# Clemapfel/egg_fluid_simulation

Hardware: AMD Instinct MI355X
Metric: pair_solves_per_sec (higher is better)
Workload: dtype f64

## Files before the change

### egg_fluid_simulation_amd/csrc/eggsim_device.h

```cpp
#pragma once
#include <stdint.h>

#define EGG_MAX_PASSES 64
#define EGG_WAVE 64

struct EggStatus {
    int32_t fail_claim;
    int32_t fail_overflow;
    int32_t fail_stall;
    int32_t fail_range;
    int32_t min_slack;
    int32_t was_cut;
    int32_t fail_levels;
    int32_t max_level;
    int32_t fail_levlds;
    int32_t reserved0;
    unsigned long long visits[EGG_MAX_PASSES];
    unsigned long long max_list;
    unsigned long long rounds;
};

struct EggStepArgs {
    const double *x_in, *y_in, *vx_in, *vy_in;
    double *x_out, *y_out, *vx_out, *vy_out;
// ... 95 lines not shown
    uint32_t *pk_ckey;
    int32_t pk_stride;
    uint32_t *lists;
    uint16_t *lvl;
    uint32_t *rank;
    uint32_t *sorted;
    uint32_t *chunks;
    int32_t *grp_nchunks;
    uint32_t *lev_start;
    int32_t *grp_nlev;
    int32_t *tile_total;
    int32_t *tile_visits;
    int32_t *tile_need;
    int32_t *tile_slack;
    int32_t *tile_fast;
    int32_t lcap, scap, lev_cap, sort_cap, chunk_cap;
    int32_t nmax, amax, ccap, use_grid, stage_cap;
    double sub_delta, damping, follow_compliance, collision_compliance, overlap_factor, cell_size, eps;
    int32_t n_substeps, n_collision_steps;
    int32_t pass_seq, substep, stale;
    int32_t tune;
    uint32_t *simd_claims;
    int32_t lev_lds_cap;
    EggStatus *status, *status_next;
};
#define EGG_PK_MAX_PASSES 64
#define EGG_PK_WINDOW 128

static inline size_t egg_pk_lists_lds_bytes(int nmax, int amax, int ccap, int use_grid, int stage_cap, int gens) {
    size_t n = (size_t)nmax, a = (size_t)amax, c = (size_t)ccap, b = 0, G = (size_t)gens;
    b += egg_align16(G * n * 4);
    b += egg_align16(G * c * 4);
    b += egg_align16(use_grid ? 0 : G * c * 4);
    b += egg_align16((n + 1) * 4);
    b += egg_align16(n * 4);
    b += egg_align16(a * 4 * 4);
    b += egg_align16((a + 1) * 4);
    b += egg_align16(16 * 4);
    b += egg_align16(G * n * 2);
    b += egg_align16(n * 2);
    {
        const size_t stage = egg_align16(((size_t)stage_cap + 1) * (n + 1) * 2), tmp = egg_align16(n * 4) + egg_align16(n * 2);
        b += stage > tmp ? stage : tmp;
    }
    return b;
}
// ... 751 lines not shown
```

### egg_fluid_simulation_amd/csrc/eggsim_host.h

```cpp
#pragma once
#include <hip/hip_runtime.h>

#include <algorithm>
#include <chrono>
#include <cmath>
#include <cstdarg>
#include <cstdio>
#include <cstdlib>
#include <cstring>
#include <functional>
#include <limits>
#include <memory>
#include <numeric>
#include <string>
#include <vector>

#include "../../include/eggsim.h"
#include "eggsim_device.h"

extern "C" __global__ void egg_step_kernel(EggStepArgs A);
extern "C" __global__ void egg_step_kernel_gl(EggStepArgs A);
extern "C" __global__ void egg_step_kernel_occ(EggStepArgs A);
extern "C" __global__ void egg_step_kernel_wide(EggStepArgs A);
extern "C" __global__ void egg_env_bounds_kernel(const double *, const double *, const double *, const double *, const double *, int,
// ... 207 lines not shown
    int nmax = 0, amax = 0, ccap = 0, use_grid = 0, lcap = 0;
    int global_lists = 0;
    int global_state = 0;
    int threads = 0;
    int wide = 0;
    int pair_cache = 0;
    size_t scratch_stride = 0;
    size_t lds = 0, scratch_offset = 0;
    int packed = -1;
};

struct PackedClass {
    int cls = 0;
    int n_tiles = 0, n_groups = 0;
    int p_begin = 0, p_end = 0;
    int tile_base = 0;
    int group_base = 0;
    size_t meta_tile_geo = 0, meta_grp_geo = 0;
    int max_group_particles = 0;
    int fused_pass = 0;
    size_t lds_pass = 0;
    int lev_lds_cap = 0;
    int lev_lds_now = 0;
    size_t lds_levels_now = 0, lds_pass_now = 0;
    int max_tiles_in_group = 0;
    int levels_ooo = 0;
    int levels_threads = 64;
    int lcap = 0, scap = 0;
    int stage_cap = 0;
    int sort_cap = 0;
    size_t sort_base = 0;
    int chunk_cap = 0;
    size_t chunk_base = 0;
    size_t lds_sort = 0;
    size_t entry_base = 0;
    size_t lds_lists = 0, lds_lists_stale = 0, lds_levels = 0, lds_exec = 0;
    int threads_lists = 64, threads_lists_stale = 64;
};

struct RelaxedBufs {
    DevBuf<double2> pos, pos_next, prev, spos, swr;
    DevBuf<int32_t> pslot, tmp, sidx, p_atom;
    DevBuf<unsigned long long> hkey, status;
    DevBuf<uint32_t> hcount, hstart;
    DevBuf<double> targets;
    DevBuf<unsigned char> scan_tmp;
    size_t scan_bytes = 0;
    uint32_t table = 0;
    uint64_t atoms_gen = ~0ull;
// ... 60 lines not shown
    int single_tile = 0;
    int uncut_streak = 0;
    double list_factor = 6.0;
    size_t list_min = 0;
    bool has_env = false;
    double env_min_mass = 0, env_max_mass = 0, env_min_radius = 0, env_max_radius = 0;
    double tiled_cell_size = 0;
    double step_follow_compliance = 57.6, step_damping = 0.9;
    int step_substeps = 2;
    bool pk_allowed = true;
    std::vector<PackedClass> pk;
    std::vector<int32_t> pk_meta_host;
    DevBuf<int32_t> pk_meta, pk_src, pk_atom, pk_tile, pk_nchunks;
    DevBuf<double> pk_pos, pk_prev, pk_wr;
    DevBuf<uint32_t> pk_ckey, pk_lists, pk_rank, pk_sorted, pk_levstart, pk_chunks;
    size_t pk_chunk_words = 0;
    DevBuf<uint16_t> pk_lvl, pk_aslot;
    size_t pk_meta_claims = 0;
    int pk_n = 0, pk_tiles = 0, pk_groups = 0;
    size_t pk_entries = 0;
    size_t pk_sort_words = 0;
    int pk_lev_cap = 255;
    int pk_seen_levels = 0;
    unsigned long long pk_seen_list = 0;
    size_t pk_lev_lds_min = 0;
    bool pk_plan_dirty = true;
    struct PkStamp { hipEvent_t a, b; int kind, launches; };
    std::vector<PkStamp> pk_stamps;
    size_t pk_stamps_used = 0;
    EggStatus *h_status = nullptr;
    RelaxedBufs rx;
    hipStream_t stream = nullptr;
    hipEvent_t ev0 = nullptr, ev1 = nullptr;
};

constexpr size_t kStatInts = 160;
static_assert(sizeof(EggStatus) <= kStatInts * 4, "status block too small");
inline EggStatus *d_stat(System &s, int parity) { return (EggStatus *)(s.d_out.p + parity * kStatInts); }
inline int32_t *d_aabb(System &s) { return s.d_out.p + 2 * kStatInts; }
inline int32_t *d_disp(System &s) { return s.d_out.p + 2 * kStatInts + 4 * s.atoms.size(); }

}
namespace egghost {
struct WireStep;
struct DrawSource;
struct InstanceState;
struct SensorState;
struct ProbeState;
// ... 221 lines not shown
int for_each_requested_atom(egg_handle *h, const char *name, int mask, int64_t n_ids, const int64_t *ids, Fn fn) {
    const std::vector<int32_t> atom_of = atom_of_batch(h);
    for (int64_t i = 0; i < n_ids; ++i) {
        const int32_t a = atom_of[(size_t)(find_batch(h, ids[i]) - h->batches.data())];
        for (int w = 0; w < 2; ++w) {
            if (!(mask >> w & 1) || a < 0) continue;
            const Atom &at = h->sys[w].atoms[(size_t)a];
            if (at.count < 1) continue;
            if (at.offset < 0 || (int64_t)at.offset + at.count > h->sys[w].n)
                return fail(h, EGG_ERR_INTERNAL, "%s: atom %d of type %d holds %d particles from %d", name, (int)a, w, (int)at.count, (int)at.offset);
            const int rc = fn(at, w, (int32_t)(2 * i + w));
            if (rc != EGG_OK) return rc;
        }
    }
    return EGG_OK;
}
typedef egg_sensor egg_region;
int check_region(egg_handle *h, const char *what, int32_t k, egg_region &o);
double cell_size_of(const egg_config &c);
int fetch_end_aabb(egg_handle *h, System &s);

extern double g_retile_ms[8];
int retile(egg_handle *h, int which);

struct Env {
    double sub_delta, damping, follow_c, collision_c, budget, cell;
    double cohesion_c;
};
Env make_env(const egg_config &c, double sub_delta, int64_t n);
enum { kWhole = 0, kPrepare = 1, kBegin = 2, kEnd = 3 };
int do_step(egg_handle *h, double delta, int S, int C, int phase = kWhole);
int follow_config(egg_handle *h, int w, bool launch);

constexpr int64_t kRelaxedMaxParticles = (int64_t)1 << 29;
#define EGG_RX_TOO_MANY_TEXT "relaxed order: more than 2^29 particles of one type"
constexpr char kRelaxedBadCellText[] = "relaxed order: a position is NaN or its spatial-hash cell lies outside +-2^30";
struct RelaxedLayout {
    size_t P = 0, nq = 0;
    bool halo = false;
    bool cohesion = false;
    bool colliders = false;
    bool forces = false;
    size_t V = 0;
    bool surfaces = false;
    bool walls = false;
    bool motion = false;
// ... 86 lines not shown
```

### egg_fluid_simulation_amd/csrc/eggsim_host_step.hip

```cpp
#include "eggsim_host.h"

namespace egghost {


Env make_env(const egg_config &c, double sub_delta, int64_t n) {
    Env e;
    e.sub_delta = sub_delta;
    auto compliance = [&](double strength) {
        double alpha = 1 - clampd(strength, 0, 1);
        return alpha / (sub_delta * sub_delta);
    };
    e.damping = 1 - clampd(c.damping, 0, 1);
    e.follow_c = compliance(c.follow_strength);
    e.collision_c = compliance(c.collision_strength);
    e.cohesion_c = compliance(c.cohesion_strength);
    double nn = (double)n;
    e.budget = c.max_collision_fraction * (nn * nn);
    e.cell = cell_size_of(c);
    return e;
}

int launch_prologue(egg_handle *h, int which, hipStream_t stream) {
    System &s = h->sys[which];
    s.parity ^= 1;
// ... 152 lines not shown
    A.scap = pc.scap;
    A.lev_cap = s.pk_lev_cap;
    A.sort_cap = pc.sort_cap;
    A.chunk_cap = pc.chunk_cap;
    A.stage_cap = pc.stage_cap;
    A.nmax = lc.nmax;
    A.amax = lc.amax;
    A.ccap = lc.ccap;
    A.use_grid = lc.use_grid;
    if (!lc.use_grid) h->stats.cell_hash[which]++;
    A.sub_delta = env.sub_delta;
    A.damping = env.damping;
    A.follow_compliance = env.follow_c;
    A.collision_compliance = env.collision_c;
    A.overlap_factor = s.cfg.collision_overlap_factor;
    A.cell_size = env.cell;
    A.eps = s.cfg.eps;
    A.n_substeps = S;
    A.n_collision_steps = C;
    A.status = d_stat(s, s.parity);
    A.status_next = d_stat(s, s.parity ^ 1);
    A.tune = h->opt_tune;
    A.lev_lds_cap = pc.lev_lds_now;
    A.simd_claims = h->simd_claims.p;
}

int launch_packed(egg_handle *h, int which, const Env &env, int S, int C) {
    System &s = h->sys[which];
    const hipStream_t st = s.stream;
    if (s.pk_plan_dirty) {
        HIP_TRY(h, hipMemcpyAsync(s.pk_meta.p, s.pk_meta_host.data(), s.pk_meta_host.size() * sizeof(int32_t),
                                  hipMemcpyHostToDevice, st));
    }
    for (PackedClass &pc : s.pk) {
        if (!pc.levels_ooo) continue;
        int now = pc.lev_lds_cap;
        if (s.pk_seen_list) now = (int)std::min<size_t>((size_t)now, std::max<size_t>((size_t)(s.pk_seen_list + s.pk_seen_list / 4 + 256), s.pk_lev_lds_min));
        now = std::min(pc.lev_lds_cap, (now + 7) & ~7);
        pc.lev_lds_now = now;
        pc.lds_levels_now = egg_pk_levels_ooo_lds_bytes(s.pk_lev_cap, pc.max_group_particles, pc.max_tiles_in_group, now);
        pc.lds_pass_now = std::max(pc.lds_levels_now, pc.lds_exec + 64 * 16 + (size_t)EGG_PK_RING_BYTES);
    }
    std::vector<EggPackedArgs> args(s.pk.size());
    for (size_t k = 0; k < s.pk.size(); ++k) fill_packed_args(h, which, s.pk[k], env, S, C, args[k]);
    const bool stamp = h->opt_timing >= 2;
    s.pk_stamps_used = 0;
    auto stamp_begin = [&](int kind) -> System::PkStamp * {
        if (!stamp) return nullptr;
        if (s.pk_stamps_used == s.pk_stamps.size()) {
            System::PkStamp ps{nullptr, nullptr, 0, 0};
            if (hipEventCreate(&ps.a) != hipSuccess || hipEventCreate(&ps.b) != hipSuccess) return nullptr;
            s.pk_stamps.push_back(ps);
        }
        System::PkStamp *ps = &s.pk_stamps[s.pk_stamps_used++];
        ps->kind = kind;
        ps->launches = (int)s.pk.size();
        (void)hipEventRecord(ps->a, st);
        return ps;
    };
    auto launch_some = [&](int take, int kind, auto kernel_of, auto grid_of, auto block_of, auto lds_of) {
        System::PkStamp *ps = nullptr;
        for (size_t k = 0; k < s.pk.size(); ++k) {
            const PackedClass &pc = s.pk[k];
// ... 327 lines not shown
                return fail(h, EGG_ERR_INTERNAL, "pair scheduler stalled (type %d, %s)", w,
                            st.fail_stall == 2 ? "time limit reached"
                            : st.fail_stall == 3 ? "workgroup narrower than the wide kernel needs"
                            : st.fail_stall == 4 ? "a wait between the waves of the packed pipeline did not end"
                                                 : "a particle's pair sequence did not finish");
            if (st.fail_overflow) {
                s.list_min = std::max<size_t>(s.list_min, (size_t)(st.max_list * 5 / 4 + 64));
                s.list_factor *= 1.5;
                if (s.list_min > (size_t)kMaxGlobalListEntries)
                    return fail(h, EGG_ERR_UNSUPPORTED, "a tile visits %llu pairs in one pass; limit is %d",
                                (unsigned long long)st.max_list, kMaxGlobalListEntries);
                s.tiling_dirty = true;
                redo = true;
                continue;
            }
            if (st.fail_levlds) {
                s.pk_lev_lds_min = std::max<size_t>(s.pk_lev_lds_min, (size_t)(st.max_list * 5 / 4 + 256));
                s.pk_seen_list = std::max(s.pk_seen_list, st.max_list);
                s.tiling_dirty = true;
                redo = true;
                continue;
            }
            if (st.fail_levels) {
                s.pk_lev_cap = std::max(2 * s.pk_lev_cap + 1, st.max_level + 64);
                if (s.pk_lev_cap > 65535)
                    return fail(h, EGG_ERR_UNSUPPORTED, "a pair-dependency chain of %d levels in one pass; limit is 65535", st.max_level);
                s.tiling_dirty = true;
                redo = true;
                continue;
            }
            if (st.fail_claim || st.fail_range) {
                std::vector<int32_t> failed(s.atoms.size());
                if (!failed.empty()) {
                    HIP_TRY(h, hipMemcpyAsync(failed.data(), s.d_atom_fail.p, failed.size() * sizeof(int32_t),
                                              hipMemcpyDeviceToHost, s.stream));
                    HIP_TRY(h, hipStreamSynchronize(s.stream));
                }
                s.extra_margin.resize(h->batches.size(), 0);
                bool any = false;
                for (size_t k = 0; k < failed.size(); ++k)
                    if (failed[k]) {
                        int &e = s.extra_margin[(size_t)s.atoms[k].batch];
                        e = std::min(4096, std::max(2, 2 * e));
                        any = true;
                    }
                if (!any) s.margin = std::min(s.margin + std::max(2, s.margin / 2), 4096);
// ... 15 lines not shown
                        break;
                    }
            }
        }
        if (redo) {
            h->stats.redo_steps++;
            continue;
        }
        for (int w = 0; w < 2; ++w) {
            System &s = h->sys[w];
            if (s.n == 0 || s.classes.empty()) continue;
            const EggStatus &st = *s.h_status;
            s.cur ^= 1;
            const int np = std::min(S * C, EGG_MAX_PASSES);
            int64_t most = 0;
            for (int p = 0; p < np; ++p) {
                h->stats.pair_solves += (int64_t)st.visits[p];
                most = std::max(most, (int64_t)st.visits[p]);
            }
            h->stats.max_pass_visits[w] = most;
            h->stats.max_levels[w] = s.pk.empty() ? 0 : st.max_level;
            if (!s.pk.empty()) {
                s.pk_seen_list = st.max_list;
                s.pk_seen_levels = st.max_level;
                s.pk_lev_lds_min = 0;
            }
#ifdef EGG_PROFILE
            if (getenv("EGGSIM_DEBUG") && !s.pk.empty())
                fprintf(stderr, "eggsim: type %d step %lld, last pass, egg_pk_levels_ooo cycles: group 0 init %llu rank %llu walk %llu finish %llu sort %llu total %llu | slowest group: walk %llu total %llu | turns %llu levels %d\n",
                        w, (long long)h->stats.steps, st.visits[55], st.visits[56], st.visits[57], st.visits[58], st.visits[59], st.visits[60], st.visits[61], st.visits[62], st.rounds, st.max_level);
            if (getenv("EGGSIM_DEBUG") && !s.pk.empty()) {
                fprintf(stderr, "   group 0 wave 0: %llu turns; cycles waiting for the batch's entries %llu, in the batch set-up %llu, in the turns %llu\n", st.visits[38], st.visits[36], st.visits[39], st.visits[37]);
                fprintf(stderr, "   executor of group 0: %llu cycles for %llu chunks = %.1f per chunk; slowest group %.1f per chunk\n", st.visits[30], st.visits[31],
                        (double)st.visits[30] / (double)std::max<unsigned long long>(st.visits[31], 1), (double)st.visits[32] / 16.0);
                fprintf(stderr, "   executor of group 0: %llu ticks of the 100 MHz clock, i.e. the cycle counter ran at %.0f MHz\n", st.visits[28], st.visits[28] ? 100.0 * (double)st.visits[30] / (double)st.visits[28] : 0.0);
                fprintf(stderr, "   executor of group 0 looked at the helper's progress %llu times and spent %llu cycles there\n", st.visits[26], st.visits[27]);
                fprintf(stderr, "   executor waves on SIMD 0 / 1 / 2 (all passes of the step): %llu %llu %llu; without a SIMD of their own: %llu\n", st.visits[33], st.visits[34], st.visits[35], st.visits[29]);
                fprintf(stderr, "   groups by total cycles (25k buckets):");
                for (int k = 0; k < 15; ++k) fprintf(stderr, " %llu", st.visits[40 + k]);
                fprintf(stderr, "\n");
            }
#endif
            h->stats.budget[w] = env[w].budget;
            h->stats.follow_solves += s.n * S;
            s.aabb_on_device = true;
            if (s.out_copied) {
                const size_t na = s.atoms.size();
                s.aabb.resize(na);
// ... 5 lines not shown
            } else {
                s.aabb_valid = false;
                s.disp_valid = false;
            }
            if (st.min_slack < std::max(1, s.margin - 1) || s.swept) s.tiling_dirty = true;
            if (s.padded && ++s.since_tiling >= 8) s.tiling_dirty = true;
            if (s.margin > h->opt_margin) {
                s.margin -= 1;
                s.tiling_dirty = true;
            }
            for (int &e : s.extra_margin)
                if (e > 0) {
                    e -= 1;
                    s.tiling_dirty = true;
                }
            if (s.single_tile && !h->opt_force_single) {
                s.uncut_streak = st.was_cut ? 0 : s.uncut_streak + 1;
                if (s.uncut_streak >= 8) {
                    s.single_tile = 0;
                    s.tiling_dirty = true;
                }
            }
            h->stats.single_tile[w] = s.single_tile;
            s.eager_boxes = s.tiling_dirty || s.claims_stale || s.targets_moving;
        }
        h->stats.last_step_kernel_ms = ms;
        for (int w = 0; w < 2; ++w) {
            System &s = h->sys[w];
            h->stats.packed[w] = (int64_t)s.pk.size();
            h->stats.pk_variants[w] = 0;
            for (const PackedClass &pc : s.pk)
                h->stats.pk_variants[w] |= (pc.levels_ooo ? EGG_PK_VARIANT_LEVELS_OOO : EGG_PK_VARIANT_LEVELS_INORDER) |
                                           (pc.n_groups <= 4 * std::max(1, h->prop.multiProcessorCount) ? EGG_PK_VARIANT_EXEC_CHAIN : EGG_PK_VARIANT_EXEC) |
                                           (pc.levels_ooo ? 0 : pc.lds_sort ? EGG_PK_VARIANT_SORT_LDS : EGG_PK_VARIANT_SORT_DIRECT) |
                                           (pc.fused_pass ? EGG_PK_VARIANT_PASS_FUSED : 0);
            for (size_t k = 0; h->opt_timing >= 2 && k < s.pk_stamps_used; ++k) {
                const System::PkStamp &ps = s.pk_stamps[k];
                float t = 0;
                if (ps.kind >= 0 && hipEventElapsedTime(&t, ps.a, ps.b) == hipSuccess) {
                    h->stats.pk_kernel_ms[w][ps.kind] += (double)t;
                    h->stats.pk_kernel_launches[w][ps.kind] += ps.launches;
                }
            }
            s.pk_stamps_used = 0;
        }
        if (h->opt_timing) {
// ... 10 lines not shown
```

### egg_fluid_simulation_amd/csrc/eggsim_host_tiling.hip

```cpp
#include "eggsim_host.h"

namespace egghost {




double g_retile_ms[8];
struct RetileLap {
    std::chrono::steady_clock::time_point t = std::chrono::steady_clock::now();
    void operator()(int k) {
        const auto n = std::chrono::steady_clock::now();
        g_retile_ms[k] += std::chrono::duration<double, std::milli>(n - t).count();
        t = n;
    }
};

static size_t pk_admitted_blocks(egg_handle *h, const void *kernel, int threads, size_t lds) {
    for (const egg_handle::PkResidency &r : h->pk_residency)
        if (r.kernel == kernel && r.threads == threads && r.lds == lds) return r.blocks > 0 ? (size_t)r.blocks : SIZE_MAX;
    int blocks = 0;
    const hipError_t e = hipOccupancyMaxActiveBlocksPerMultiprocessor(&blocks, kernel, threads, lds);
    if (e != hipSuccess || blocks <= 0) {
        (void)hipGetLastError();
        blocks = 0;
        if (!h->pk_residency_warned)
            fprintf(stderr, "eggsim: no residency answer for a list kernel at %d threads, %zu B LDS (%s): thread counts are chosen by the LDS / wave model alone\n",
                    threads, lds, hipGetErrorString(e));
        h->pk_residency_warned = true;
    }
    h->pk_residency.push_back({kernel, threads, lds, blocks});
    return blocks > 0 ? (size_t)blocks : SIZE_MAX;
}

static size_t pk_lists_admitted(egg_handle *h, int gens, int threads, size_t lds) {
    const bool fold = !(h->opt_tune & 128);
    if (gens == 2)
        return pk_admitted_blocks(h, fold ? (const void *)egg_pk_lists_stale_mid_kernel : (const void *)egg_pk_lists_stale_kernel, threads, lds);
    const size_t plain = pk_admitted_blocks(h, (const void *)egg_pk_lists_fresh_kernel, threads, lds);
    return fold ? std::min(plain, pk_admitted_blocks(h, (const void *)egg_pk_lists_first_kernel, threads, lds)) : plain;
}

int retile(egg_handle *h, int which) {
    System &s = h->sys[which];
    RetileLap lap;
    int rc = upload_atoms(h, which);
    if (rc != EGG_OK) return rc;
    const size_t na = s.atoms.size();
    const double cell = cell_size_of(s.cfg);
    s.extra_margin.resize(h->batches.size(), 0);
    s.tile_atom_begin.assign(1, 0);
    s.tile_atoms.clear();
    s.classes.clear();
    h->stats.n_tiles[which] = 0;
    h->stats.max_tile_particles[which] = 0;
    if (na == 0) {
        s.tiling_dirty = false;
        s.tiled_cell_size = cell;
        return EGG_OK;
    }
    if (!s.aabb_valid && s.aabb_on_device && s.tiled_cell_size == cell) {
        rc = fetch_end_aabb(h, s);
        if (rc != EGG_OK) return rc;
// ... 408 lines not shown
            }
            const int64_t gp_max = std::max<int64_t>(h->opt_group_particles > 0 ? h->opt_group_particles : gp_auto,
                                                     tiles[(size_t)lc.first_tile].particles);
            int max_tiles_in_group = 0;
            for (int t = 0; t < lc.n_tiles;) {
                int64_t in_group = 0;
                int t_end = t;
                while (t_end < lc.n_tiles && t_end - t < 64) {
                    const int64_t np = tiles[(size_t)lc.first_tile + t_end].particles;
                    if (t_end > t && (in_group + np > gp_max || in_group + np > 32767)) break;
                    in_group += np;
                    ++t_end;
                }
                const int32_t rec[4] = {t, t_end, tile_first_particle[(size_t)t], (int32_t)in_group};
                s.pk_meta_host.insert(s.pk_meta_host.end(), rec, rec + 4);
                pc.n_groups++;
                pc.max_group_particles = std::max<int>(pc.max_group_particles, (int)in_group);
                max_tiles_in_group = std::max(max_tiles_in_group, t_end - t);
                t = t_end;
            }
            const int simds = 4 * std::max(1, h->prop.multiProcessorCount);
            const bool dense_tiles = tiles[(size_t)lc.first_tile].particles > 256;
            pc.levels_ooo = h->lds_lane_ordered && h->opt_level_walk != 1 && (h->opt_level_walk == 2 || (pc.n_groups <= simds && dense_tiles));
            if (pc.levels_ooo) {
                const size_t guess = s.pk_seen_list ? (size_t)(s.pk_seen_list * 3 / 2 + 512) : (size_t)24 * lc.nmax;
                pc.lev_lds_cap = (int)std::min<size_t>((size_t)pc.scap, std::max<size_t>(guess, s.pk_lev_lds_min));
                pc.lev_lds_cap = (pc.lev_lds_cap + 7) & ~7;
                if (pc.n_groups > std::max(1, h->prop.multiProcessorCount)) {
                    const size_t budget = (kLdsMax - 4096) / 2;
                    const size_t fixed = egg_pk_levels_ooo_lds_bytes(s.pk_lev_cap, pc.max_group_particles, max_tiles_in_group, 0);
                    if (budget > fixed) {
                        const size_t fit = ((budget - fixed) / ((size_t)max_tiles_in_group * 2)) & ~(size_t)7;
                        const size_t need = std::max<size_t>((size_t)(s.pk_seen_list + s.pk_seen_list / 16 + 64), s.pk_lev_lds_min);
                        if (fit >= need && (size_t)pc.lev_lds_cap > fit) pc.lev_lds_cap = (int)fit;
                    }
                }
                pc.levels_threads = 64 * std::min(16, std::max(4, max_tiles_in_group <= 4 ? 2 * max_tiles_in_group : max_tiles_in_group));
                pc.lds_levels = egg_pk_levels_ooo_lds_bytes(s.pk_lev_cap, pc.max_group_particles, max_tiles_in_group, pc.lev_lds_cap);
                if (pc.lds_levels > h->lds_limit) pc.levels_ooo = 0;
            }
            pc.fused_pass = pc.levels_ooo && pc.levels_threads <= 512 && max_tiles_in_group <= 4 && pc.n_groups <= simds && !(h->opt_tune & 64);
            if (!pc.levels_ooo) {
                pc.levels_threads = std::min(256, (max_tiles_in_group * 16 + 63) / 64 * 64);
                pc.lds_levels = egg_pk_levels_mr_lds_bytes(s.pk_lev_cap, pc.max_group_particles, pc.levels_threads);
            }
            const size_t sort_words = (size_t)max_tiles_in_group * (size_t)pc.scap + 64;
            pc.chunk_cap = (int)std::min<size_t>(sort_words / 64 + (size_t)s.pk_lev_cap + 8, (size_t)1 << 28);
            pc.lds_exec = (size_t)pc.max_group_particles * 16;
            pc.lds_sort = egg_align16((size_t)(s.pk_lev_cap + 2) * 4) + sort_words * 4;
            if (pc.lds_sort > 64 * 1024) pc.lds_sort = 0;
            if (pc.lds_exec + 64 * 16 > h->lds_limit || pc.lds_levels > h->lds_limit || sort_words >= ((size_t)1 << 26)) {
                s.pk_meta_host.resize(meta_mark);
                continue;
            }
            if (pc.fused_pass) {
                pc.lds_pass = std::max(pc.lds_levels, pc.lds_exec + 64 * 16 + (size_t)EGG_PK_RING_BYTES);
                if (pc.lds_pass > h->lds_limit) pc.fused_pass = 0;
            }
            pc.sort_cap = (int)sort_words;
            pc.max_tiles_in_group = max_tiles_in_group;
            pc.lev_lds_now = pc.lev_lds_cap;
            pc.lds_levels_now = pc.lds_levels;
            pc.lds_pass_now = pc.lds_pass;
            if (getenv("EGGSIM_DEBUG"))
                fprintf(stderr, "eggsim: type %d packed class: %d tiles of <= %d particles in %d groups, grid cells %d (%s), lists: %d threads, %d staged partners, %zu B LDS; levels: %s, %d threads, %zu B LDS (level array %d entries); pass fused %d, %zu B LDS\n",
                        which, lc.n_tiles, lc.nmax, pc.n_groups, lc.ccap, lc.use_grid ? "dense grid" : "hash", pc.threads_lists, pc.stage_cap, pc.lds_lists,
                        pc.levels_ooo ? "out of order" : "in order", pc.levels_threads, pc.lds_levels, pc.lev_lds_cap, pc.fused_pass, pc.lds_pass);
            pc.chunk_base = s.pk_chunk_words;
            s.pk_chunk_words += (size_t)pc.n_groups * (size_t)pc.chunk_cap;
            lc.packed = (int)s.pk.size();
            s.pk_n = pn;
            s.pk_tiles += lc.n_tiles;
            s.pk_groups += pc.n_groups;
            s.pk_entries += (size_t)lc.n_tiles * (size_t)pc.scap;
            s.pk_sort_words += (size_t)pc.n_groups * (size_t)pc.sort_cap;
            s.pk.push_back(pc);
        }
        if (!s.pk.empty()) {
            s.pk_meta_claims = (s.pk_meta_host.size() + 3) & ~(size_t)3;
            s.pk_meta_host.resize(s.pk_meta_claims);
            for (int32_t a : s.tile_atoms) {
                const Box &c = claim[(size_t)a];
                const int32_t rec[4] = {c.lo_x, c.lo_y, c.hi_x, c.hi_y};
                s.pk_meta_host.insert(s.pk_meta_host.end(), rec, rec + 4);
            }
            lap(5);
            const size_t np = (size_t)s.pk_n, nt = (size_t)s.pk_tiles, ng = (size_t)s.pk_groups;
            HIP_TRY(h, s.pk_meta.reserve(s.pk_meta_host.size() + 4, false, s.stream));
            HIP_TRY(h, s.pk_src.reserve(np, false, s.stream));
            HIP_TRY(h, s.pk_atom.reserve(np, false, s.stream));
            HIP_TRY(h, s.pk_aslot.reserve(np + 8, false, s.stream));
            HIP_TRY(h, s.pk_pos.reserve(2 * np, false, s.stream));
            HIP_TRY(h, s.pk_prev.reserve(2 * np, false, s.stream));
            HIP_TRY(h, s.pk_wr.reserve(2 * np, false, s.stream));
            HIP_TRY(h, s.pk_ckey.reserve(2 * np, false, s.stream));
            HIP_TRY(h, s.pk_lists.reserve(s.pk_entries + 64, false, s.stream));
            HIP_TRY(h, s.pk_lvl.reserve(s.pk_entries + 64, false, s.stream));
            bool any_ooo = false;
            for (const PackedClass &pc : s.pk) any_ooo |= pc.levels_ooo != 0;
            if (any_ooo) HIP_TRY(h, s.pk_rank.reserve(s.pk_entries + 64, false, s.stream));
            HIP_TRY(h, s.pk_sorted.reserve(s.pk_sort_words + 64, false, s.stream));
            HIP_TRY(h, s.pk_chunks.reserve(s.pk_chunk_words + 64, false, s.stream));
            HIP_TRY(h, s.pk_nchunks.reserve(2 * ng + 8, false, s.stream));
            HIP_TRY(h, s.pk_levstart.reserve(ng * ((size_t)s.pk_lev_cap + 2) + 64, false, s.stream));
            HIP_TRY(h, s.pk_tile.reserve(nt * (3 + 2 * EGG_PK_MAX_PASSES) + 4, false, s.stream));
        }
        s.pk_plan_dirty = true;
    }

    HIP_TRY(h, s.d_scratch.reserve(scratch_bytes + 16, false, s.stream));
    lap(6);
    s.h_claim = claim;
    s.meta_dirty = true;
    s.tiling_dirty = false;
    h->stats.retiles++;
    h->stats.n_tiles[which] = (int64_t)tiles.size();
    h->stats.max_tile_particles[which] = tiles.empty() ? 0 : tiles.front().particles;
    lap(7);
    return EGG_OK;
}

}
```

### egg_fluid_simulation_amd/csrc/eggsim_packed.hip

```cpp
#include <hip/hip_runtime.h>
#include "eggsim_device.h"

#include "eggsim_tile.h"

namespace {


__device__ inline uint32_t pk_cell_meta(const Tile &t, int gh, int buf, uint32_t key) {
    if (t.use_grid) return t.cell(buf)[(int)(key >> 16) * gh + (int)(key & 0xFFFFu)];
    return cell_meta(t, buf, key);
}

template <class F>
__device__ inline int pk_visit_fresh(const Tile &t, int gh, int cur, int i, F emit) {
    const uint32_t ki = t.ckey(cur)[i];
    const uint16_t *items = t.hitems(cur);
    int count = 0;
    if (t.use_grid) {
        const uint32_t *cells = t.cell(cur);
        const int h1 = (int)(ki >> 16) * gh + (int)(ki & 0xFFFFu);
#pragma unroll
        for (int p = 0; p < 3; ++p) {
            const int h0 = h1 + (p - 1) * gh - 1;
            const uint32_t m0 = cells[h0], m2 = cells[h0 + 2];
// ... 397 lines not shown
            } else {
                pk_visit_fresh(t, gh, cur, i, emit);
            }
        }
    }
#pragma unroll
    for (int d = 32; d >= 1; d >>= 1) guarded += __shfl_xor(guarded, d, 64);
    if ((tid & 63) == 0) wtot[tid >> 6] = guarded;
    __syncthreads();
    if (tid == 0) {
        uint32_t gsum = 0;
        for (int w = 0; w < (nthreads + 63) / 64; ++w) gsum += wtot[w];
        A.tile_visits[(size_t)min(A.pass_seq, EGG_PK_MAX_PASSES - 1) * A.n_tiles + tile] =
            (fits && !any_bad) ? total - (int)gsum : 0;
    }
}
#define EGG_PK_LISTS_KERNEL extern "C" __global__ void __launch_bounds__(1024) __attribute__((amdgpu_num_sgpr(72)))
EGG_PK_LISTS_KERNEL egg_pk_lists_fresh_kernel(EggPackedArgs A) { egg_pk_lists_body<false, false>(A, blockIdx.x); }
EGG_PK_LISTS_KERNEL egg_pk_lists_stale_kernel(EggPackedArgs A) { egg_pk_lists_body<true, false>(A, blockIdx.x); }
EGG_PK_LISTS_KERNEL egg_pk_lists_first_kernel(EggPackedArgs A) { egg_pk_lists_body<false, true>(A, blockIdx.x); }
EGG_PK_LISTS_KERNEL egg_pk_lists_stale_mid_kernel(EggPackedArgs A) { egg_pk_lists_body<true, true>(A, blockIdx.x); }


__device__ __forceinline__ bool pk_levels_finish(const EggPackedArgs &A, int g, const uint32_t *hist, int maxlev, bool over, int lane, uint32_t *cursor = nullptr) {
    const int lev_cap = A.lev_cap;
    if (over && lane == 0) atomicExch(&A.status->fail_levels, 1);
    if (lane == 0 && maxlev > __hip_atomic_load(&A.status->max_level, __ATOMIC_RELAXED, __HIP_MEMORY_SCOPE_AGENT))
        atomicMax(&A.status->max_level, maxlev);
    const int nlev = min(maxlev, lev_cap);
    uint32_t *lstart = A.lev_start + (size_t)g * (lev_cap + 2);
    uint32_t *chunks = A.chunks + (size_t)g * A.chunk_cap;
    uint32_t carry = 0, ccarry = 0;
    for (int b0 = 1; b0 <= nlev; b0 += 64) {
        const int L = b0 + lane;
        const uint32_t v = (L <= nlev) ? hist[L] : 0u;
        const uint32_t nch = (v + 63u) >> 6;
        const uint32_t incl = (uint32_t)wave_incl_scan((int)v, lane), cincl = (uint32_t)wave_incl_scan((int)nch, lane);
        const uint32_t start = carry + incl - v, cb = ccarry + cincl - nch;
        if (L <= nlev) {
            lstart[L] = start;
            if (cursor) cursor[L] = start;
            for (uint32_t c = 0; c < nch; ++c)
                if (cb + c < (uint32_t)A.chunk_cap) chunks[cb + c] = (start + 64u * c) | ((min(64u, v - 64u * c) - 1u) << 26);
        }
        carry += (uint32_t)__builtin_amdgcn_readlane((int)incl, 63);
        ccarry += (uint32_t)__builtin_amdgcn_readlane((int)cincl, 63);
    }
    const bool usable = !over && ccarry <= (uint32_t)A.chunk_cap && carry <= (uint32_t)A.sort_cap;
    if (lane == 0) {
        lstart[nlev + 1] = carry;
        A.grp_nchunks[g] = usable ? (int)ccarry : 0;
        A.grp_nlev[g] = usable ? nlev : 0;
// ... 110 lines not shown
                const bool run_ends = (sl == m - 1) || ((heads >> (sl + 1)) & 1u);
                last[base + b] = (uint16_t)l;
                lv[q + r + sl] = (uint16_t)l;
                atomicAdd(&hist[l], 1u);
                maxlev = max(maxlev, l);
                if (run_ends) last[base + a] = (uint16_t)l;
            }
            r += m;
        }
    }
#pragma unroll
    for (int d = 32; d >= 1; d >>= 1) maxlev = max(maxlev, __shfl_xor(maxlev, d, 64));
    over = __any(over);
    if (lane == 0) {
        wave_max[tid >> 6] = maxlev;
        wave_over[tid >> 6] = over ? 1 : 0;
    }
    __syncthreads();
    if (tid >= 64) return;
    for (int w = 0; w < nthreads / 64; ++w) {
        maxlev = max(maxlev, wave_max[w]);
        over = over || wave_over[w];
    }
    pk_levels_finish(A, g, hist, maxlev, over, lane);
}

#ifdef EGG_PROFILE
#define EGG_STAMP(name) const unsigned long long name = __builtin_amdgcn_s_memtime()
#else
#define EGG_STAMP(name)
#endif

__device__ __forceinline__ void pk_levels_ooo_body(const EggPackedArgs &A, const int g, const int nthreads) {
    extern __shared__ __align__(16) unsigned char smem[];
    EGG_STAMP(TS);
    if (g >= A.n_groups) return;
    const int tid = threadIdx.x, lane = tid & 63, wave = tid >> 6, nwaves = nthreads >> 6;
    const int4 gg = ((const int4 *)A.grp_geo)[g];
    const int t0 = __builtin_amdgcn_readfirstlane(gg.x), t1 = __builtin_amdgcn_readfirstlane(gg.y);
    const int p0 = __builtin_amdgcn_readfirstlane(gg.z), np = __builtin_amdgcn_readfirstlane(gg.w);
    const int nt = t1 - t0;
    const int lev_cap = A.lev_cap;
    uint32_t *hist = (uint32_t *)smem;
    unsigned char *q8 = smem + egg_align16((size_t)(lev_cap + 2) * 4);
    uint32_t *word = (uint32_t *)q8;
    q8 += egg_align16((size_t)np * 4);
    uint32_t *cnt = (uint32_t *)q8;
    q8 += egg_align16((size_t)(np + 64) * 4);
    uint32_t *cnt2 = (uint32_t *)q8;
    q8 += egg_align16((size_t)(np + 64) * 4);
    uint16_t *llv = (uint16_t *)q8;
    const int lcap_lds = A.lev_lds_cap;
    __shared__ int tile_base[64], tile_len[64], tile_half[64];
    __shared__ int wave_max[16], wave_over[16];
    for (int i = tid; i <= lev_cap + 1; i += nthreads) hist[i] = 0;
    for (int i = tid; i < np + 64; i += nthreads) {
        if (i < np) word[i] = 0;
        cnt[i] = 0;
        cnt2[i] = 0;
    }
    const bool split_rank = 2 * nt <= nwaves;
    if (tid < nt) {
        tile_base[tid] = ((const int4 *)A.tile_geo)[2 * (t0 + tid)].x - p0;
        int slen = A.tile_total[t0 + tid];
        if (slen > lcap_lds) {
// ... 169 lines not shown
        }
    }
    over = maxlev > lev_cap || turns >= EGG_PK_SPIN_LIMIT;
    if (turns >= EGG_PK_SPIN_LIMIT && lane == 0) atomicExch(&A.status->fail_stall, 4);
    EGG_STAMP(T3);
#pragma unroll
    for (int d = 32; d >= 1; d >>= 1) maxlev = max(maxlev, __shfl_xor(maxlev, d, 64));
    over = __any(over);
    if (lane == 0) {
        wave_max[wave] = maxlev;
        wave_over[wave] = over ? 1 : 0;
        atomicMax(&A.status->rounds, (unsigned long long)turns);
    }
    __syncthreads();
    EGG_STAMP(T3b);
    __shared__ int usable_s;
    if (tid < 64) {
        for (int w = 0; w < nwaves; ++w) {
            maxlev = max(maxlev, wave_max[w]);
            over = over || wave_over[w];
        }
        bool lds_ok = true;
        for (int t = 0; t < nt; ++t) lds_ok = lds_ok && A.tile_total[t0 + t] <= lcap_lds;
        const bool usable = pk_levels_finish(A, g, hist, maxlev, over || !lds_ok, lane, hist) && lds_ok;
        if (lane == 0) usable_s = usable ? 1 : 0;
    }
    __syncthreads();
    EGG_STAMP(T4);
    if (!usable_s) return;
    uint32_t *sorted = A.sorted + (size_t)g * A.sort_cap;
    for (int t = 0; t < nt; ++t) {
        const uint32_t base = (uint32_t)tile_base[t];
        const int slen = tile_len[t];
        const uint32_t *stream = A.lists + (size_t)(t0 + t) * A.scap;
        const uint16_t *lv = llv + (size_t)t * lcap_lds;
        for (int e0 = 0; e0 < slen; e0 += 32 * nthreads) {
            uint32_t rec[32];
#pragma unroll
            for (int u = 0; u < 32; ++u) rec[u] = stream[min(e0 + u * nthreads + tid, slen - 1)];
            uint32_t pos[32];
#pragma unroll
            for (int u = 0; u < 32; ++u) {
                const int e = e0 + u * nthreads + tid;
                const bool valid = e < slen;
                const uint32_t l = (uint32_t)lv[min(e, slen - 1)];
                pos[u] = __hip_atomic_fetch_add(&hist[l], valid ? 1u : 0u, __ATOMIC_RELAXED, __HIP_MEMORY_SCOPE_WORKGROUP);
            }
// ... 670 lines not shown
```

Baseline: 12.00 billion.

## Size level histogram from observed depth and grow level tables ahead of need

The out-of-order level kernel now sizes its LDS level histogram from the recently observed maximum level plus headroom, rather than from the full level cap. This shrinks LDS use and can raise occupancy. When the histogram overflows, the step is redone with a larger histogram minimum before the global level cap is grown. After each step the level tables are also grown ahead of need based on how fast level depth is rising, reusing a factored-out sizing routine, which avoids costly failed passes and retiles. The cost is more redo paths and host bookkeeping.

Result: slower. 11.21 billion (-6.6%).

```diff
diff --git a/egg_fluid_simulation_amd/csrc/eggsim_device.h b/egg_fluid_simulation_amd/csrc/eggsim_device.h
--- a/egg_fluid_simulation_amd/csrc/eggsim_device.h
+++ b/egg_fluid_simulation_amd/csrc/eggsim_device.h
@@ -141,6 +141,7 @@
     int32_t tune;
     uint32_t *simd_claims;
     int32_t lev_lds_cap;
+    int32_t lev_hist_cap;
     EggStatus *status, *status_next;
 };
 #define EGG_PK_MAX_PASSES 64
diff --git a/egg_fluid_simulation_amd/csrc/eggsim_host.h b/egg_fluid_simulation_amd/csrc/eggsim_host.h
--- a/egg_fluid_simulation_amd/csrc/eggsim_host.h
+++ b/egg_fluid_simulation_amd/csrc/eggsim_host.h
@@ -253,9 +253,11 @@
     size_t lds_pass = 0;
     int lev_lds_cap = 0;
     int lev_lds_now = 0;
+    int lev_hist_now = 0;
     size_t lds_levels_now = 0, lds_pass_now = 0;
     int max_tiles_in_group = 0;
     int levels_ooo = 0;
+    int levels_ooo_wanted = 0;
     int levels_threads = 64;
     int lcap = 0, scap = 0;
     int stage_cap = 0;
@@ -362,8 +364,11 @@
     size_t pk_sort_words = 0;
     int pk_lev_cap = 255;
     int pk_seen_levels = 0;
+    int pk_prev_levels = 0;
     unsigned long long pk_seen_list = 0;
     size_t pk_lev_lds_min = 0;
+    int pk_hist_min = 0;
+    int pk_hist_now = 0;
     bool pk_plan_dirty = true;
     struct PkStamp { hipEvent_t a, b; int kind, launches; };
     std::vector<PkStamp> pk_stamps;
@@ -631,6 +636,7 @@
 
 extern double g_retile_ms[8];
 int retile(egg_handle *h, int which);
+int grow_level_tables(egg_handle *h, int which, int rise);
 
 struct Env {
     double sub_delta, damping, follow_c, collision_c, budget, cell;
diff --git a/egg_fluid_simulation_amd/csrc/eggsim_host_step.hip b/egg_fluid_simulation_amd/csrc/eggsim_host_step.hip
--- a/egg_fluid_simulation_amd/csrc/eggsim_host_step.hip
+++ b/egg_fluid_simulation_amd/csrc/eggsim_host_step.hip
@@ -198,6 +198,7 @@
     A.status_next = d_stat(s, s.parity ^ 1);
     A.tune = h->opt_tune;
     A.lev_lds_cap = pc.lev_lds_now;
+    A.lev_hist_cap = pc.lev_hist_now ? pc.lev_hist_now : s.pk_lev_cap;
     A.simd_claims = h->simd_claims.p;
 }
 
@@ -208,13 +209,19 @@
         HIP_TRY(h, hipMemcpyAsync(s.pk_meta.p, s.pk_meta_host.data(), s.pk_meta_host.size() * sizeof(int32_t),
                                   hipMemcpyHostToDevice, st));
     }
+    s.pk_hist_now = 0;
     for (PackedClass &pc : s.pk) {
         if (!pc.levels_ooo) continue;
+        int hist = s.pk_lev_cap;
+        if (s.pk_seen_levels) hist = std::min(hist, std::max(s.pk_seen_levels + s.pk_seen_levels / 4 + 64, s.pk_hist_min));
+        hist = std::min(s.pk_lev_cap, ((hist + 2 + 3) & ~3) - 2);
         int now = pc.lev_lds_cap;
         if (s.pk_seen_list) now = (int)std::min<size_t>((size_t)now, std::max<size_t>((size_t)(s.pk_seen_list + s.pk_seen_list / 4 + 256), s.pk_lev_lds_min));
         now = std::min(pc.lev_lds_cap, (now + 7) & ~7);
+        pc.lev_hist_now = hist;
+        s.pk_hist_now = s.pk_hist_now ? std::min(s.pk_hist_now, hist) : hist;
         pc.lev_lds_now = now;
-        pc.lds_levels_now = egg_pk_levels_ooo_lds_bytes(s.pk_lev_cap, pc.max_group_particles, pc.max_tiles_in_group, now);
+        pc.lds_levels_now = egg_pk_levels_ooo_lds_bytes(hist, pc.max_group_particles, pc.max_tiles_in_group, now);
         pc.lds_pass_now = std::max(pc.lds_levels_now, pc.lds_exec + 64 * 16 + (size_t)EGG_PK_RING_BYTES);
     }
     std::vector<EggPackedArgs> args(s.pk.size());
@@ -588,6 +595,11 @@
                 continue;
             }
             if (st.fail_levels) {
+                if (s.pk_hist_now && s.pk_hist_now < s.pk_lev_cap) {
+                    s.pk_hist_min = std::max(2 * s.pk_hist_now + 1, st.max_level + st.max_level / 4 + 64);
+                    redo = true;
+                    continue;
+                }
                 s.pk_lev_cap = std::max(2 * s.pk_lev_cap + 1, st.max_level + 64);
                 if (s.pk_lev_cap > 65535)
                     return fail(h, EGG_ERR_UNSUPPORTED, "a pair-dependency chain of %d levels in one pass; limit is 65535", st.max_level);
@@ -649,8 +661,10 @@
             h->stats.max_levels[w] = s.pk.empty() ? 0 : st.max_level;
             if (!s.pk.empty()) {
                 s.pk_seen_list = st.max_list;
+                s.pk_prev_levels = attempt == 0 ? s.pk_seen_levels : 0;
                 s.pk_seen_levels = st.max_level;
                 s.pk_lev_lds_min = 0;
+                s.pk_hist_min = 0;
             }
 #ifdef EGG_PROFILE
             if (getenv("EGGSIM_DEBUG") && !s.pk.empty())
@@ -702,6 +716,10 @@
                 }
             }
             h->stats.single_tile[w] = s.single_tile;
+            if (!s.pk.empty()) {
+                const int rc = grow_level_tables(h, w, s.pk_prev_levels > 0 ? s.pk_seen_levels - s.pk_prev_levels : 0);
+                if (rc != EGG_OK) return rc;
+            }
             s.eager_boxes = s.tiling_dirty || s.claims_stale || s.targets_moving;
         }
         h->stats.last_step_kernel_ms = ms;
diff --git a/egg_fluid_simulation_amd/csrc/eggsim_host_tiling.hip b/egg_fluid_simulation_amd/csrc/eggsim_host_tiling.hip
--- a/egg_fluid_simulation_amd/csrc/eggsim_host_tiling.hip
+++ b/egg_fluid_simulation_amd/csrc/eggsim_host_tiling.hip
@@ -38,6 +38,85 @@
         return pk_admitted_blocks(h, fold ? (const void *)egg_pk_lists_stale_mid_kernel : (const void *)egg_pk_lists_stale_kernel, threads, lds);
     const size_t plain = pk_admitted_blocks(h, (const void *)egg_pk_lists_fresh_kernel, threads, lds);
     return fold ? std::min(plain, pk_admitted_blocks(h, (const void *)egg_pk_lists_first_kernel, threads, lds)) : plain;
+}
+
+static bool size_level_tables(const egg_handle *h, const System &s, int lev_cap, int nmax, PackedClass &pc) {
+    const int simds = 4 * std::max(1, h->prop.multiProcessorCount);
+    const int max_tiles_in_group = pc.max_tiles_in_group;
+    pc.lds_pass = 0;
+    if (pc.levels_ooo) {
+        const size_t guess = s.pk_seen_list ? (size_t)(s.pk_seen_list * 3 / 2 + 512) : (size_t)24 * nmax;
+        pc.lev_lds_cap = (int)std::min<size_t>((size_t)pc.scap, std::max<size_t>(guess, s.pk_lev_lds_min));
+        pc.lev_lds_cap = (pc.lev_lds_cap + 7) & ~7;
+        if (pc.n_groups > std::max(1, h->prop.multiProcessorCount)) {
+            const size_t budget = (kLdsMax - 4096) / 2;
+            const size_t fixed = egg_pk_levels_ooo_lds_bytes(lev_cap, pc.max_group_particles, max_tiles_in_group, 0);
+            if (budget > fixed) {
+                const size_t fit = ((budget - fixed) / ((size_t)max_tiles_in_group * 2)) & ~(size_t)7;
+                const size_t need = std::max<size_t>((size_t)(s.pk_seen_list + s.pk_seen_list / 16 + 64), s.pk_lev_lds_min);
+                if (fit >= need && (size_t)pc.lev_lds_cap > fit) pc.lev_lds_cap = (int)fit;
+            }
+        }
+        pc.levels_threads = 64 * std::min(16, std::max(4, max_tiles_in_group <= 4 ? 2 * max_tiles_in_group : max_tiles_in_group));
+        pc.lds_levels = egg_pk_levels_ooo_lds_bytes(lev_cap, pc.max_group_particles, max_tiles_in_group, pc.lev_lds_cap);
+        if (pc.lds_levels > h->lds_limit) pc.levels_ooo = 0;
+    }
+    pc.fused_pass = pc.levels_ooo && pc.levels_threads <= 512 && max_tiles_in_group <= 4 && pc.n_groups <= simds && !(h->opt_tune & 64);
+    if (!pc.levels_ooo) {
+        pc.levels_threads = std::min(256, (max_tiles_in_group * 16 + 63) / 64 * 64);
+        pc.lds_levels = egg_pk_levels_mr_lds_bytes(lev_cap, pc.max_group_particles, pc.levels_threads);
+    }
+    const size_t sort_words = (size_t)max_tiles_in_group * (size_t)pc.scap + 64;
+    pc.chunk_cap = (int)std::min<size_t>(sort_words / 64 + (size_t)lev_cap + 8, (size_t)1 << 28);
+    pc.lds_exec = (size_t)pc.max_group_particles * 16;
+    pc.lds_sort = egg_align16((size_t)(lev_cap + 2) * 4) + sort_words * 4;
+    if (pc.lds_sort > 64 * 1024) pc.lds_sort = 0;
+    if (pc.lds_exec + 64 * 16 > h->lds_limit || pc.lds_levels > h->lds_limit || sort_words >= ((size_t)1 << 26)) return false;
+    if (pc.fused_pass) {
+        pc.lds_pass = std::max(pc.lds_levels, pc.lds_exec + 64 * 16 + (size_t)EGG_PK_RING_BYTES);
+        if (pc.lds_pass > h->lds_limit) pc.fused_pass = 0;
+    }
+    pc.sort_cap = (int)sort_words;
+    pc.lev_lds_now = pc.lev_lds_cap;
+    pc.lds_levels_now = pc.lds_levels;
+    pc.lds_pass_now = pc.lds_pass;
+    return true;
+}
+
+static int reserve_level_tables(egg_handle *h, System &s) {
+    HIP_TRY(h, s.pk_chunks.reserve(s.pk_chunk_words + 64, false, s.stream));
+    HIP_TRY(h, s.pk_levstart.reserve((size_t)s.pk_groups * ((size_t)s.pk_lev_cap + 2) + 64, false, s.stream));
+    return EGG_OK;
+}
+
+int grow_level_tables(egg_handle *h, int which, int rise) {
+    System &s = h->sys[which];
+    if (s.pk.empty()) return EGG_OK;
+    const int64_t headroom = std::max<int64_t>(64, 8 * (int64_t)std::max(0, rise));
+    const int cap = 2 * s.pk_lev_cap + 1;
+    if ((int64_t)s.pk_seen_levels + headroom <= (int64_t)s.pk_lev_cap || cap > 65535) return EGG_OK;
+    if (s.tiling_dirty) {
+        s.pk_lev_cap = cap;
+        return EGG_OK;
+    }
+    std::vector<PackedClass> next = s.pk;
+    size_t chunk_words = 0;
+    for (PackedClass &pc : next) {
+        const int was_ooo = pc.levels_ooo, was_fused = pc.fused_pass;
+        pc.levels_ooo = pc.levels_ooo_wanted;
+        if (!size_level_tables(h, s, cap, s.classes[(size_t)pc.cls].nmax, pc) || pc.levels_ooo != was_ooo || pc.fused_pass != was_fused) {
+            s.pk_lev_cap = cap;
+            s.tiling_dirty = true;
+            return EGG_OK;
+        }
+        pc.chunk_base = chunk_words;
+        chunk_words += (size_t)pc.n_groups * (size_t)pc.chunk_cap;
+    }
+    s.pk = std::move(next);
+    s.pk_chunk_words = chunk_words;
+    s.pk_lev_cap = cap;
+    if (getenv("EGGSIM_DEBUG")) fprintf(stderr, "eggsim: type %d level tables grown to %d levels ahead of need (%d seen, +%d in the last step)\n", which, cap, s.pk_seen_levels, rise);
+    return reserve_level_tables(h, s);
 }
 
 int retile(egg_handle *h, int which) {
@@ -492,46 +571,12 @@
             const int simds = 4 * std::max(1, h->prop.multiProcessorCount);
             const bool dense_tiles = tiles[(size_t)lc.first_tile].particles > 256;
             pc.levels_ooo = h->lds_lane_ordered && h->opt_level_walk != 1 && (h->opt_level_walk == 2 || (pc.n_groups <= simds && dense_tiles));
-            if (pc.levels_ooo) {
-                const size_t guess = s.pk_seen_list ? (size_t)(s.pk_seen_list * 3 / 2 + 512) : (size_t)24 * lc.nmax;
-                pc.lev_lds_cap = (int)std::min<size_t>((size_t)pc.scap, std::max<size_t>(guess, s.pk_lev_lds_min));
-                pc.lev_lds_cap = (pc.lev_lds_cap + 7) & ~7;
-                if (pc.n_groups > std::max(1, h->prop.multiProcessorCount)) {
-                    const size_t budget = (kLdsMax - 4096) / 2;
-                    const size_t fixed = egg_pk_levels_ooo_lds_bytes(s.pk_lev_cap, pc.max_group_particles, max_tiles_in_group, 0);
-                    if (budget > fixed) {
-                        const size_t fit = ((budget - fixed) / ((size_t)max_tiles_in_group * 2)) & ~(size_t)7;
-                        const size_t need = std::max<size_t>((size_t)(s.pk_seen_list + s.pk_seen_list / 16 + 64), s.pk_lev_lds_min);
-                        if (fit >= need && (size_t)pc.lev_lds_cap > fit) pc.lev_lds_cap = (int)fit;
-                    }
-                }
-                pc.levels_threads = 64 * std::min(16, std::max(4, max_tiles_in_group <= 4 ? 2 * max_tiles_in_group : max_tiles_in_group));
-                pc.lds_levels = egg_pk_levels_ooo_lds_bytes(s.pk_lev_cap, pc.max_group_particles, max_tiles_in_group, pc.lev_lds_cap);
-                if (pc.lds_levels > h->lds_limit) pc.levels_ooo = 0;
-            }
-            pc.fused_pass = pc.levels_ooo && pc.levels_threads <= 512 && max_tiles_in_group <= 4 && pc.n_groups <= simds && !(h->opt_tune & 64);
-            if (!pc.levels_ooo) {
-                pc.levels_threads = std::min(256, (max_tiles_in_group * 16 + 63) / 64 * 64);
-                pc.lds_levels = egg_pk_levels_mr_lds_bytes(s.pk_lev_cap, pc.max_group_particles, pc.levels_threads);
-            }
-            const size_t sort_words = (size_t)max_tiles_in_group * (size_t)pc.scap + 64;
-            pc.chunk_cap = (int)std::min<size_t>(sort_words / 64 + (size_t)s.pk_lev_cap + 8, (size_t)1 << 28);
-            pc.lds_exec = (size_t)pc.max_group_particles * 16;
-            pc.lds_sort = egg_align16((size_t)(s.pk_lev_cap + 2) * 4) + sort_words * 4;
-            if (pc.lds_sort > 64 * 1024) pc.lds_sort = 0;
-            if (pc.lds_exec + 64 * 16 > h->lds_limit || pc.lds_levels > h->lds_limit || sort_words >= ((size_t)1 << 26)) {
+            pc.levels_ooo_wanted = pc.levels_ooo;
+            pc.max_tiles_in_group = max_tiles_in_group;
+            if (!size_level_tables(h, s, s.pk_lev_cap, lc.nmax, pc)) {
                 s.pk_meta_host.resize(meta_mark);
                 continue;
             }
-            if (pc.fused_pass) {
-                pc.lds_pass = std::max(pc.lds_levels, pc.lds_exec + 64 * 16 + (size_t)EGG_PK_RING_BYTES);
-                if (pc.lds_pass > h->lds_limit) pc.fused_pass = 0;
-            }
-            pc.sort_cap = (int)sort_words;
-            pc.max_tiles_in_group = max_tiles_in_group;
-            pc.lev_lds_now = pc.lev_lds_cap;
-            pc.lds_levels_now = pc.lds_levels;
-            pc.lds_pass_now = pc.lds_pass;
             if (getenv("EGGSIM_DEBUG"))
                 fprintf(stderr, "eggsim: type %d packed class: %d tiles of <= %d particles in %d groups, grid cells %d (%s), lists: %d threads, %d staged partners, %zu B LDS; levels: %s, %d threads, %zu B LDS (level array %d entries); pass fused %d, %zu B LDS\n",
                         which, lc.n_tiles, lc.nmax, pc.n_groups, lc.ccap, lc.use_grid ? "dense grid" : "hash", pc.threads_lists, pc.stage_cap, pc.lds_lists,
@@ -570,9 +615,11 @@
             for (const PackedClass &pc : s.pk) any_ooo |= pc.levels_ooo != 0;
             if (any_ooo) HIP_TRY(h, s.pk_rank.reserve(s.pk_entries + 64, false, s.stream));
             HIP_TRY(h, s.pk_sorted.reserve(s.pk_sort_words + 64, false, s.stream));
-            HIP_TRY(h, s.pk_chunks.reserve(s.pk_chunk_words + 64, false, s.stream));
             HIP_TRY(h, s.pk_nchunks.reserve(2 * ng + 8, false, s.stream));
-            HIP_TRY(h, s.pk_levstart.reserve(ng * ((size_t)s.pk_lev_cap + 2) + 64, false, s.stream));
+            {
+                const int rc = reserve_level_tables(h, s);
+                if (rc != EGG_OK) return rc;
+            }
             HIP_TRY(h, s.pk_tile.reserve(nt * (3 + 2 * EGG_PK_MAX_PASSES) + 4, false, s.stream));
         }
         s.pk_plan_dirty = true;
diff --git a/egg_fluid_simulation_amd/csrc/eggsim_packed.hip b/egg_fluid_simulation_amd/csrc/eggsim_packed.hip
--- a/egg_fluid_simulation_amd/csrc/eggsim_packed.hip
+++ b/egg_fluid_simulation_amd/csrc/eggsim_packed.hip
@@ -443,12 +443,12 @@
 EGG_PK_LISTS_KERNEL egg_pk_lists_stale_mid_kernel(EggPackedArgs A) { egg_pk_lists_body<true, true>(A, blockIdx.x); }
 
 
-__device__ __forceinline__ bool pk_levels_finish(const EggPackedArgs &A, int g, const uint32_t *hist, int maxlev, bool over, int lane, uint32_t *cursor = nullptr) {
+__device__ __forceinline__ bool pk_levels_finish(const EggPackedArgs &A, int g, const uint32_t *hist, int maxlev, bool over, int lane, uint32_t *cursor, int hist_cap) {
     const int lev_cap = A.lev_cap;
     if (over && lane == 0) atomicExch(&A.status->fail_levels, 1);
     if (lane == 0 && maxlev > __hip_atomic_load(&A.status->max_level, __ATOMIC_RELAXED, __HIP_MEMORY_SCOPE_AGENT))
         atomicMax(&A.status->max_level, maxlev);
-    const int nlev = min(maxlev, lev_cap);
+    const int nlev = min(maxlev, hist_cap);
     uint32_t *lstart = A.lev_start + (size_t)g * (lev_cap + 2);
     uint32_t *chunks = A.chunks + (size_t)g * A.chunk_cap;
     uint32_t carry = 0, ccarry = 0;
@@ -605,7 +605,7 @@
         maxlev = max(maxlev, wave_max[w]);
         over = over || wave_over[w];
     }
-    pk_levels_finish(A, g, hist, maxlev, over, lane);
+    pk_levels_finish(A, g, hist, maxlev, over, lane, nullptr, lev_cap);
 }
 
 #ifdef EGG_PROFILE
@@ -623,7 +623,7 @@
     const int t0 = __builtin_amdgcn_readfirstlane(gg.x), t1 = __builtin_amdgcn_readfirstlane(gg.y);
     const int p0 = __builtin_amdgcn_readfirstlane(gg.z), np = __builtin_amdgcn_readfirstlane(gg.w);
     const int nt = t1 - t0;
-    const int lev_cap = A.lev_cap;
+    const int lev_cap = min(A.lev_hist_cap, A.lev_cap);
     uint32_t *hist = (uint32_t *)smem;
     unsigned char *q8 = smem + egg_align16((size_t)(lev_cap + 2) * 4);
     uint32_t *word = (uint32_t *)q8;
@@ -839,7 +839,7 @@
         }
         bool lds_ok = true;
         for (int t = 0; t < nt; ++t) lds_ok = lds_ok && A.tile_total[t0 + t] <= lcap_lds;
-        const bool usable = pk_levels_finish(A, g, hist, maxlev, over || !lds_ok, lane, hist) && lds_ok;
+        const bool usable = pk_levels_finish(A, g, hist, maxlev, over || !lds_ok, lane, hist, lev_cap) && lds_ok;
         if (lane == 0) usable_s = usable ? 1 : 0;
     }
     __syncthreads();
```
